# daisy9542/yolo-puncture

Hardware: AMD Instinct MI355X
Metric: images/sec (higher is better)
Workload: dtype bf16

## Files before the change

### include/yolop.h

```cpp
#ifndef YOLOP_H
#define YOLOP_H

#include <stddef.h>
#include <stdint.h>

#ifdef __cplusplus
extern "C" {
#endif

#define YP_OK 0
#define YP_ERR_ARG -1
#define YP_ERR_STATE -2
#define YP_ERR_HIP -3
#define YP_ERR_WEIGHT -4

#define YP_BF16 0
#define YP_F32 1

#define YP_TASK_DETECT 0
#define YP_TASK_SEGMENT 1

#define YP_NM 32
#define YP_MAX_MASKS 480
#define YP_MAX_DET 512
// ... 83 lines not shown

typedef struct yp_cls yp_cls;
int yp_cls_create(int variant, int dtype, int device, yp_cls** out);
int yp_cls_destroy(yp_cls* e);
int yp_cls_weight_count(const yp_cls* e);
int yp_cls_weight_info(const yp_cls* e, int i, char* name, int name_cap, int64_t shape[4], int* ndim);
int yp_cls_set_weight(yp_cls* e, const char* name, const float* host, const int64_t* shape, int ndim);
int yp_cls_finalize(yp_cls* e);
int yp_cls_forward(yp_cls* e, const uint8_t* frames_dev, int B, int H, int W, int bgr, const int32_t* boxes_dev, float* logits_out,
                   float* prob_out, int32_t* cls_out, void* stream);
int yp_cls_set_graph(yp_cls* e, int enable);
int yp_cls_tensor_count(const yp_cls* e);
int yp_cls_tensor_info(const yp_cls* e, int i, char* name, int name_cap, int dims[4] );
int yp_cls_tensor_read(yp_cls* e, int i, float* host_out);

typedef struct yp_comm yp_comm;
int yp_comm_unique_id(void* id128);
int yp_comm_create(const void* id128, int rank, int world, int device, yp_comm** out);
int yp_allgather(yp_comm* c, const void* send_dev, void* recv_dev, size_t bytes_per_rank, void* stream);
int yp_comm_destroy(yp_comm* c);

#define YP_MAX_ANCHORS 294912
int yp_max_batch(const yp_engine* e, int H, int W);
int yp_plan(yp_engine* e, int B, int H, int W);
int yp_op_info(const yp_engine* e, int i, char* name, int name_cap, int* kind, double* flops,
               double* bytes);
int yp_op_kernel(const yp_engine* e, int i, char* name, int name_cap);
int yp_op_output(const yp_engine* e, int i, int* tensor, int* coff, int* C);
int yp_op_input(const yp_engine* e, int i, int* tensor, int* coff, int* C, int* c_read);
int yp_op_fusion(const yp_engine* e, int i, int* pre, int* pre_stored);
int yp_debug_op_form(const yp_engine* e, int i, int* form, int* absorbed, int cap);
int yp_run_op(yp_engine* e, int i, const uint8_t* in_dev, float* det_out, int32_t* idx_out, float* coeff_out, void* stream);
int yp_tensor_write(yp_engine* e, int tensor, int coff, int C, const float* host);
int yp_tensor_count(const yp_engine* e);
int yp_tensor_info(const yp_engine* e, int i, char* name, int name_cap, int dims[4] , int* is_f32);
int yp_tensor_read(yp_engine* e, int i, float* host_out);

int yp_profile(yp_engine* e, const uint8_t* in_dev, int B, int H, int W, float* det_out, int32_t* idx_out,
               float* coeff_out, float* ms_out, int iters, void* stream);

int yp_set_nms(yp_engine* e, float conf, float iou);

int yp_set_attention_form(yp_engine* e, int form);

int yp_set_autotune(yp_engine* e, int enable);

int yp_tuning_export(const yp_engine* e, int32_t* cfg_out, int cap);
int yp_tuning_import(yp_engine* e, int B, int H, int W, const int32_t* cfg, int n);

int yp_debug_force_conv_cfg(int cfg);
int yp_debug_op_cfg(const yp_engine* e, int i, int* cfg);
int yp_debug_last_store_form(void);
int yp_debug_max_workgroups(int n);
int yp_debug_conv_families(int* base, int* num_cfgs, int cap);
int yp_debug_ablation(int v);
int yp_debug_head_clocks(uint64_t* out8);
int yp_debug_attention(const void* qkv_dev, void* o_dev, int dtype, int B, int N, int nh, int kd, int hd, int q_stride, int q_coff, int o_stride,
                       int o_coff, int wgs, int* kernel_out, void* stream);
int yp_debug_attention_form(const void* qkv_dev, void* o_dev, int dtype, int B, int N, int nh, int kd, int hd, int q_stride, int q_coff, int o_stride,
                            int o_coff, int wgs, int form, int* kernel_out, void* stream);
int yp_debug_topk_anchors(const uint32_t* const mk_dev[3], int B, const int hw[3][2], int k, int32_t* sel_out_dev, uint32_t* thr_out_dev, void* stream);
int yp_debug_head_branch_clocks(uint64_t* out8);
int yp_debug_head_winners(yp_engine* e, int32_t* sel_host, float* box_host, float* coeff_host);
int yp_debug_contour_clocks(uint64_t* out12);
int yp_debug_pwsp_clocks(uint64_t* out32);

int yp_tuning_source(const yp_engine* e);

int yp_debug_host_selftest(yp_engine* e);
int yp_debug_graph_info(const yp_engine* e, int64_t* out6);
int yp_debug_head_positions(yp_engine* e, int64_t* out6);
int yp_debug_marker(void* stream);

int yp_set_graph(yp_engine* e, int enable);

#ifdef __cplusplus
}
#endif
#endif
```

### yolo-puncture_amd/csrc/common.h

```cpp
#pragma once
#include <hip/hip_runtime.h>
#include <stdint.h>
#include <atomic>
#include <cstdlib>
#include <string>
#include <vector>

namespace yp {

enum DType { DT_BF16 = 0, DT_F32 = 1 };
enum Act { ACT_NONE = 0, ACT_SILU = 1, ACT_RELU = 2 };

enum OpKind {
    OP_STEM = 0,
    OP_CONV = 1,
    OP_DWCONV = 2,
    OP_POOL5 = 3,
    OP_UPSAMPLE = 4,
    OP_ATTN = 5,
    OP_HEAD = 6,
    OP_CONVT = 7,
    OP_AMAX = 9,
    OP_POOL3 = 8,
};
// ... 103 lines not shown
    const float* bias;
    void* y; int y_stride, y_coff; int Ho, Wo;
    const void* res; int res_stride, res_coff;
    int B, ks, stride, pad, act;
    int gs, gstride;
    size_t x_bytes;
};

struct StemParams {
    const uint8_t* x; int H, W;
    const float* w;
    const void* wpk;
    const float* bias;
    void* y; int y_stride, y_coff; int Ho, Wo, C0; int B;
    int act;
};

struct FrontParams {
    const uint8_t* img; int imgH, imgW, B;
    const void* w0; const float* bias0; int act0, C0; int H1, W1;
    const void* w1; const float* bias1; int act1, C1, Kpad1; size_t w1_bytes;
    const void* w2; const float* bias2; int act2, C2, Kpad2; size_t w2_bytes;
    void* y; int y_stride, y_coff; size_t y_bytes; int Ho, Wo;
    unsigned long long* clk;
};
bool frontend_valid(const FrontParams& p);
hipError_t launch_frontend(const FrontParams& p, hipStream_t st);

struct C2fParams {
    const void* x; int x_stride, x_coff; size_t x_bytes;
    int B, H, W, C;
    const void* w1; const float* bias1; int act1, Kpad1; size_t w1_bytes;
    const void* w2; const float* bias2; int act2, Kpad2; size_t w2_bytes;
    int shortcut;
    const void* w3; const float* bias3; int act3, Kpad3, Cout; size_t w3_bytes;
    void* y; int y_stride, y_coff; size_t y_bytes;
    unsigned long long* clk;
    int wide;
};
bool c2f_fused_valid(const C2fParams& p);

struct ScdParams {
    const void* x; int x_stride, x_coff; size_t x_bytes; int B, H, W, K;
    const void* w1; const float* bias1; int act1, Kpad1, C; size_t w1_bytes;
    const void* wd; const float* biasd; int actd;
    void* y; int y_stride, y_coff; size_t y_bytes; int Ho, Wo;
    unsigned long long* clk;
};
bool scdown_fused_valid(const ScdParams& p);
const char* scdown_fused_kernel_name(const ScdParams& p);
bool scdown_stream_valid(const ScdParams& p);
const char* scdown_stream_kernel_name(const ScdParams& p);
hipError_t launch_scdown_stream(const ScdParams& p, hipStream_t st);
hipError_t launch_scdown_fused(const ScdParams& p, hipStream_t st);
hipError_t launch_c2f_fused(const C2fParams& p, hipStream_t st);

struct PoolParams {
    const void* x; int x_stride, x_coff;
    void* y; int y_stride, y_coff;
    int B, H, W, C;
};

struct UpParams {
    const void* x; int x_stride, x_coff;
    void* y; int y_stride, y_coff;
    int B, H, W, C;
};

struct AttnParams {
    const void* qkv; int q_stride, q_coff;
    void* o; int o_stride, o_coff;
    int B, N, nh, kd, hd;
    float scale;
};

struct HeadParams {
    const float* box[3]; const float* cls[3]; const float* cf[3];
    int hw[3][2]; int nlev;
    int B, nc, max_det, A;
    float* det; int32_t* idx; float* coeff;
    void* scratch;
    const unsigned* mk[3];
    const float* nms_params;
    float* nms_ws;
    int* sp_sel; int* sp_wlist; int* sp_wcount; unsigned* sp_thr; float* sp_box; float* sp_cf;
    int* sp_plist; int* sp_pcount; int sp_plist_off[3], sp_plist_cap[3];
};
hipError_t launch_head_stage1(const HeadParams& p, hipStream_t st);
hipError_t launch_head_stage2(const HeadParams& p, hipStream_t st);
constexpr int HEAD_MAXK = 512;
struct HeadBranchParams {
    const void* x[3]; int x_stride[3], x_coff[3], H[3], W[3], Cin[3]; size_t x_bytes[3];
    const void* w0[3]; int Kpad0[3]; const float* b0[3];
    const void* w1[3]; int Kpad1[3]; const float* b1[3];
    const void* w2[3]; int Kpad2[3]; const float* b2[3];
    int act0, act1;
    int B, max_det, maxk, cmid, cout;
    int A0, A1;
    const int* sel;
    const int* wlist;
    const int* wcount;
    float* out;
    const int* plist; const int* pcount;
    int plist_off[3], plist_cap[3];
    void* t0; size_t t0_off[3], t0_bytes;
    int pos_grid;
// ... 206 lines not shown
```

### yolo-puncture_amd/csrc/engine.hip

```cpp
#include "../../include/yolop.h"
#include "common.h"
#include <algorithm>
#include <array>
#include <chrono>

#include <cmath>
#include <cstdarg>
#include <cstdio>
#include <cstring>
#include <cstdlib>
#include <dlfcn.h>
#include <fcntl.h>
#include <fstream>
#include <map>
#include <sstream>
#include <memory>

using namespace yp;

static thread_local char g_err[512] = "";
static int fail(int code, const char* fmt, ...) {
    va_list ap;
    va_start(ap, fmt);
    vsnprintf(g_err, sizeof(g_err), fmt, ap);
// ... 2390 lines not shown
    HIPCHK(hipSetDevice(e->device));
    HIPCHK(hipDeviceSynchronize());
    const SparseWs ws = sparse_ws_layout(*e);
    const char* base = (const char*)e->sp_ws;
    int pc[8];
    HIPCHK(hipMemcpy(pc, base + ws.pcount, sizeof(pc), hipMemcpyDeviceToHost));
    std::vector<int> wc((size_t)e->pB * 3);
    HIPCHK(hipMemcpy(wc.data(), base + ws.wcount, wc.size() * 4, hipMemcpyDeviceToHost));
    for (int l = 0; l < 3; ++l) {
        out6[l] = std::min(pc[4 + l], ws.plist_cap[l]);
        for (int b = 0; b < e->pB; ++b) out6[3 + l] += wc[(size_t)b * 3 + l];
    }
    return 1;
}

__global__ void op_marker_kernel(int* sink) { if (sink) *sink = 0; }
int yp_debug_marker(void* stream) {
    hipLaunchKernelGGL(op_marker_kernel, dim3(1), dim3(1), 0, (hipStream_t)stream, (int*)nullptr);
    HIPCHK(hipGetLastError());
    return YP_OK;
}

int yp_debug_pwsp_clocks(uint64_t* out32) {
    if (!out32) return fail(YP_ERR_ARG, "yp_debug_pwsp_clocks: null output");
    HIPCHK(hipDeviceSynchronize());
    HIPCHK(pwsp_read_clocks((unsigned long long*)out32));
    return YP_OK;
}

int yp_debug_contour_clocks(uint64_t* out12) {
    if (!out12) return fail(YP_ERR_ARG, "yp_debug_contour_clocks: null output");
    HIPCHK(hipDeviceSynchronize());
    HIPCHK(contour_read_clocks((unsigned long long*)out12));
    return YP_OK;
}

int yp_debug_ablation(int v) {
    conv_set_debug_ablation(v);
    return 0;
}

int yp_debug_force_conv_cfg(int cfg) {
    conv_dma_force_cfg(cfg);
    return conv_dma_family.num_cfgs;
}

int yp_debug_last_store_form(void) {
    store_form_watched().store(true);
    return last_store_form().exchange(-1);
}

int yp_debug_max_workgroups(int n) { return debug_max_workgroups_ref().exchange(n > 0 ? n : 0); }

int yp_debug_op_cfg(const yp_engine* e, int i, int* cfg) {
    if (!e || i < 0 || i >= (int)e->ops.size() || !cfg) return fail(YP_ERR_ARG, "bad argument");
    *cfg = op_launch_cfg(*e, e->ops[i]);
    return YP_OK;
}

int yp_debug_conv_families(int* base, int* num_cfgs, int cap) {
    for (int f = 0; f < kNumConvFamilies && f < cap; ++f) {
        if (base) base[f] = kConvFamilies[f]->base;
        if (num_cfgs) num_cfgs[f] = kConvFamilies[f]->num_cfgs;
    }
    return kNumConvFamilies;
}

int yp_debug_host_selftest(yp_engine* e) {
    if (!e) return fail(YP_ERR_ARG, "null engine");
    if (!e->planned) return fail(YP_ERR_STATE, "yp_plan has not been called");
    size_t acc = 0;
    if (!e->finalized)
        for (WeightDesc& w : e->weights) {
            if (!w.have_w || !w.have_b || w.w.empty()) continue;
            std::vector<unsigned char> main, aux;
            pack_weight(*e, w, main, aux);
            acc += main.size() + aux.size();
        }
    for (const Op& o : e->ops) {
        if (o.skip) continue;
        if (fused(o)) build_form_params(*e, o);
        else if (o.kind == OP_CONV) acc += (size_t)conv_params(*e, o).Cout;
    }
    save_tune_cache(*e);
    (void)load_tune_cache(*e);
    {
        const std::string tp = tune_cache_path(*e, true);
        if (!tp.empty() && std::ifstream(tp).good()) {
            std::vector<std::pair<int, std::string>> keep;
            for (const Op& o : e->ops) keep.emplace_back(o.cfg, o.kernel);
            const bool ok = load_tune_cache(*e, true);
            for (size_t i = 0; i < e->ops.size(); ++i) { e->ops[i].cfg = keep[i].first; e->ops[i].kernel = keep[i].second; }
            if (!ok) return fail(YP_ERR_STATE, "packaged tune table %s does not apply to this build's plan", tp.c_str());
        }
    }
    remember_tuning(*e);
    if (!recall_tuning(*e)) return fail(YP_ERR_STATE, "internal: tuning memo lost");
    int rc = build_lane_schedule(*e);
    if (rc != YP_OK) return rc;
    std::vector<char> rec(e->ops.size(), 0);
    std::vector<char> seen(e->n_lanes, 0);
    seen[0] = 1;
    for (const auto& stp : e->lane_steps) {
        const Op& o = e->ops[stp.op];
        for (int j : stp.waits)
            if (!rec[j]) return fail(YP_ERR_STATE, "internal: %s waits on %s, which never records", o.name.c_str(), e->ops[j].name.c_str());
// ... 264 lines not shown
```

### yolo-puncture_amd/csrc/scdown_fused.hip

```cpp
#include "common.h"
#include <cstdio>
#include <cstdlib>
#include <vector>

namespace yp {

constexpr int SD_NW = 8;
constexpr int SD_TH = 4, SD_TW = 8;
constexpr int SD_RH = 2 * SD_TH + 1, SD_RW = 2 * SD_TW + 1;
constexpr int SD_RP = SD_RH * SD_RW;
constexpr int SD_XP = 39;
constexpr int SD_XB = SD_XP * 1024;
constexpr int SD_TB = 160 * 128;
constexpr int SD_WB = 64 * 256;
constexpr int SD_LDS = 2 * SD_XB + 2 * SD_TB + 2 * SD_WB + 5120 + 2048;

__global__ __launch_bounds__(SD_NW * 64) void scdown_fused_kernel(const ScdParams p, const int tiles_h, const int tiles_w, const int G) {
    extern __shared__ __attribute__((aligned(1024))) unsigned char smem[];
    unsigned char* const Xs = smem;
    unsigned char* const Ts = Xs + 2 * SD_XB;
    unsigned char* const Ws = Ts + 2 * SD_TB;
    unsigned char* const Wd = Ws + 2 * SD_WB;
    float* const Bs = (float*)(Wd + 5120);

// ... 109 lines not shown
            SD_STAMP(3)

            {
                bf16x8 wA[4], xB[2][5];
                int q[5];
#pragma unroll
                for (int kc = 0; kc < 4; ++kc) { const int row = cf * 16 + fr; wA[kc] = *(const bf16x8*)(Wg + row * 256 + (((kc * 4 + fc) ^ (row & 15)) * 16)); }
#pragma unroll
                for (int j = 0; j < 5; ++j) { const int qq = (ps + 2 * j) * 16 + fr; q[j] = qq < SD_XP * 4 ? qq : SD_XP * 4 - 1; }
                auto rd = [&](int kc) {
#pragma unroll
                    for (int j = 0; j < 5; ++j) xB[kc & 1][j] = *(const bf16x8*)(X + q[j] * 256 + (((kc * 4 + fc) ^ (q[j] & 15)) * 16));
                };
                f32x4 acc[5];
                const f32x4 b1 = *(const f32x4*)(Bs + g * 64 + cf * 16 + fc * 4);
#pragma unroll
                for (int j = 0; j < 5; ++j) acc[j] = b1;
                rd(0);
                __builtin_amdgcn_sched_barrier(0);
#pragma unroll
                for (int kc = 0; kc < 4; ++kc) {
                    if (kc < 3) rd(kc + 1);
#pragma unroll
                    for (int j = 0; j < 5; ++j) acc[j] = __builtin_amdgcn_mfma_f32_16x16x32_bf16(wA[kc], xB[kc & 1][j], acc[j], 0, 0, 0);
                    __builtin_amdgcn_sched_barrier(0);
                }
#pragma unroll
                for (int j = 0; j < 5; ++j) {
                    const int qq = (ps + 2 * j) * 16 + fr;
                    const int py = q[j] / SD_RW, px = q[j] - py * SD_RW;
                    const int iy = 2 * th * SD_TH - 1 + py, ix = 2 * tw * SD_TW - 1 + px;
                    const bool in = (unsigned)iy < (unsigned)p.H && (unsigned)ix < (unsigned)p.W;
                    float v[4] = {acc[j][0], acc[j][1], acc[j][2], acc[j][3]};
                    if (p.act1 == ACT_SILU) silu4_packed(v);
                    __attribute__((aligned(8))) __bf16 ob[4];
#pragma unroll
                    for (int i = 0; i < 4; ++i) ob[i] = (__bf16)(in ? v[i] : 0.f);
                    const int ch = cf * 16 + fc * 4;
                    lds_write8(Tg + qq * 128 + (((ch >> 3) ^ ((qq >> 1) & 7)) * 16) + (ch & 7) * 2, *(const unsigned long long*)ob);
                }
            }
            asm volatile("s_waitcnt lgkmcnt(0)" ::: "memory");
            SD_STAMP(2)
            pg = g; pb = b; pth = th; ptw = tw;
        }
    }
    __builtin_amdgcn_s_barrier();
    if (pg >= 0) dw_stage(Ts + ((gi - 1) & 1) * SD_TB, pg, pb, pth, ptw);
    __builtin_amdgcn_s_waitcnt(0 | (7 << 4) | (0xF << 8));
    if (p.clk && lane == 0)
        for (int i = 0; i < 4; ++i) p.clk[((size_t)blockIdx.x * SD_NW + wave) * 4 + i] = clk[i];
}

const char* scdown_fused_kernel_name(const ScdParams& p) { return scdown_stream_valid(p) ? scdown_stream_kernel_name(p) : "scdown_fused_kernel"; }

bool scdown_fused_valid(const ScdParams& p) {
    if (scdown_stream_valid(p)) return true;
    if (p.K != 128 || p.Kpad1 != 128 || (p.C & 63) || p.C > 256 || p.C < 64) return false;
    if ((p.x_stride & 7) || (p.x_coff & 7) || (p.y_stride & 3) || (p.y_coff & 3)) return false;
    if (p.x_bytes >= (1ull << 31) || p.y_bytes >= (1ull << 31)) return false;
    if (p.w1_bytes < (size_t)p.C * p.Kpad1 * 2) return false;
    if ((p.H & 1) || (p.W & 1) || p.Ho * 2 != p.H || p.Wo * 2 != p.W) return false;
    const long covered = (long)((p.Ho + SD_TH - 1) / SD_TH * SD_TH) * ((p.Wo + SD_TW - 1) / SD_TW * SD_TW);
    if (covered * 2 > (long)p.Ho * p.Wo * 3) return false;
    return true;
}

hipError_t launch_scdown_fused(const ScdParams& p, hipStream_t st) {
    if (scdown_stream_valid(p)) return launch_scdown_stream(p, st);
    const int tiles_h = (p.Ho + SD_TH - 1) / SD_TH, tiles_w = (p.Wo + SD_TW - 1) / SD_TW;
    const int num_tiles = p.B * tiles_h * tiles_w;
    int G = 256;
    if (G > num_tiles) G = num_tiles;
    static size_t granted = 0;
    if (hipError_t e = allow_dynamic_lds((const void*)scdown_fused_kernel, (size_t)SD_LDS, granted)) return e;
    static const bool clocks = env_on("YOLOP_SCD_CLOCKS");
    if (clocks) {
        ScdParams q = p;
        const size_t n = (size_t)G * SD_NW * 4;
        if (hipMalloc((void**)&q.clk, n * 8) != hipSuccess) return hipErrorOutOfMemory;
        hipLaunchKernelGGL(scdown_fused_kernel, dim3(G), dim3(SD_NW * 64), (size_t)SD_LDS, st, q, tiles_h, tiles_w, G);
        (void)hipStreamSynchronize(st);
        std::vector<unsigned long long> h(n);
        (void)hipMemcpy(h.data(), q.clk, n * 8, hipMemcpyDeviceToHost);
        (void)hipFree(q.clk);
        static const char* nm[4] = {"wait", "barrier", "G (1x1+SiLU)", "issue+D (dw)"};
        const double steps = (double)num_tiles / G * (p.C / 64);
        for (int w = 0; w < SD_NW; w += SD_NW - 1) {
            fprintf(stderr, "[scdown clocks] wave %d, s_memtime ticks per channel group:", w);
            for (int i = 0; i < 4; ++i) {
                double s = 0;
                for (int g = 0; g < G; ++g) s += (double)h[((size_t)g * SD_NW + w) * 4 + i];
                fprintf(stderr, " %s %.0f", nm[i], s / G / steps);
            }
            fprintf(stderr, "\n");
        }
        return hipGetLastError();
    }
    hipLaunchKernelGGL(scdown_fused_kernel, dim3(G), dim3(SD_NW * 64), (size_t)SD_LDS, st, p, tiles_h, tiles_w, G);
    return hipGetLastError();
}

}
```

### yolo-puncture_amd/engine.py

```python
from __future__ import annotations

import ctypes as C
import os
from typing import Dict, List, Optional, Tuple

import numpy as np
import torch

from .weights import fold_state

_LIB: Optional[C.CDLL] = None
_HERE = os.path.dirname(os.path.abspath(__file__))
LIB_PATH = os.environ.get("YOLOP_LIB") or os.path.join(_HERE, "libyolop.so")

YP_BF16, YP_F32 = 0, 1
TASK_DETECT, TASK_SEGMENT = 0, 1
OP_KINDS = {0: "stem", 1: "conv", 2: "dwconv", 3: "pool5", 4: "upsample", 5: "attn", 6: "head", 7: "convT", 8: "pool3", 9: "amax"}
FORMS = ("plain", "dwpw", "dwpw_tail", "s2pw", "frontend", "c2f", "scdown", "pwsp", "cls_out")


class ModelDesc(C.Structure):
    _fields_ = [("variant", C.c_int), ("nc", C.c_int), ("task", C.c_int), ("dtype", C.c_int), ("max_det", C.c_int), ("family", C.c_int)]


# ... 27 lines not shown
    lib.yp_mask_contours.restype = C.c_int
    lib.yp_mask_contours_scaled.argtypes = [vp, C.c_int, C.c_int, C.c_int, C.c_int, C.c_int, vp, vp, vp, C.c_int, vp, C.c_int, C.c_int, vp]
    lib.yp_mask_contours_scaled.restype = C.c_int
    lib.yp_mask_contours_large_workspace.argtypes = [C.c_int, C.c_int, C.c_int]
    lib.yp_mask_contours_large_workspace.restype = C.c_size_t
    lib.yp_mask_contours_large.argtypes = [vp, C.c_int, C.c_int, C.c_int, C.c_int, C.c_int, vp, vp, vp, C.c_int, vp, C.c_int, C.c_int, C.c_int, vp,
                                           C.c_size_t, vp]
    lib.yp_mask_contours_large.restype = C.c_int
    lib.yp_plan.argtypes = [vp, C.c_int, C.c_int, C.c_int]
    lib.yp_max_batch.argtypes = [vp, C.c_int, C.c_int]
    lib.yp_max_batch.restype = C.c_int
    lib.yp_debug_topk_anchors.argtypes = [C.POINTER(vp), C.c_int, C.POINTER(C.c_int), C.c_int, vp, vp, vp]
    lib.yp_debug_topk_anchors.restype = C.c_int
    lib.yp_debug_attention.argtypes = [vp, vp] + [C.c_int] * 11 + [ip, vp]
    lib.yp_debug_attention.restype = C.c_int
    lib.yp_debug_attention_form.argtypes = [vp, vp] + [C.c_int] * 12 + [ip, vp]
    lib.yp_debug_attention_form.restype = C.c_int
    lib.yp_set_attention_form.argtypes = [vp, C.c_int]
    lib.yp_set_attention_form.restype = C.c_int
    lib.yp_op_info.argtypes = [vp, C.c_int, C.c_char_p, C.c_int, ip, C.POINTER(C.c_double), C.POINTER(C.c_double)]
    lib.yp_op_output.argtypes = [vp, C.c_int, ip, ip, ip]
    lib.yp_op_kernel.argtypes = [vp, C.c_int, C.c_char_p, C.c_int]
    lib.yp_op_fusion.argtypes = [vp, C.c_int, ip, ip]
    lib.yp_op_fusion.restype = C.c_int
    lib.yp_debug_op_form.argtypes = [vp, C.c_int, ip, ip, C.c_int]
    lib.yp_debug_op_form.restype = C.c_int
    lib.yp_run_op.argtypes = [vp, C.c_int, vp, vp, vp, vp, vp]
    lib.yp_tensor_write.argtypes = [vp, C.c_int, C.c_int, C.c_int, vp]
    lib.yp_tensor_count.argtypes = [vp]
    lib.yp_tensor_info.argtypes = [vp, C.c_int, C.c_char_p, C.c_int, ip, ip]
    lib.yp_tensor_read.argtypes = [vp, C.c_int, vp]
    lib.yp_profile.argtypes = [vp, vp, C.c_int, C.c_int, C.c_int, vp, vp, vp, vp, C.c_int, vp]
    lib.yp_set_graph.argtypes = [vp, C.c_int]
    lib.yp_set_autotune.argtypes = [vp, C.c_int]
    lib.yp_set_nms.argtypes = [vp, C.c_float, C.c_float]
    lib.yp_set_nms.restype = C.c_int
    lib.yp_debug_host_selftest.argtypes = [vp]
    lib.yp_debug_host_selftest.restype = C.c_int
    lib.yp_tuning_source.argtypes = [vp]
    lib.yp_tuning_source.restype = C.c_int
    lib.yp_debug_graph_info.argtypes = [vp, C.POINTER(C.c_int64)]
    lib.yp_debug_graph_info.restype = C.c_int
    lib.yp_debug_head_positions.argtypes = [vp, C.POINTER(C.c_int64)]
    lib.yp_debug_head_positions.restype = C.c_int
    lib.yp_debug_marker.argtypes = [vp]
    lib.yp_debug_marker.restype = C.c_int
    lib.yp_debug_force_conv_cfg.argtypes = [C.c_int]
    lib.yp_debug_op_cfg.argtypes = [vp, C.c_int, ip]
    lib.yp_debug_op_cfg.restype = C.c_int
    lib.yp_debug_last_store_form.argtypes = []
    lib.yp_debug_last_store_form.restype = C.c_int
    lib.yp_debug_max_workgroups.argtypes = [C.c_int]
    lib.yp_debug_max_workgroups.restype = C.c_int
    lib.yp_debug_conv_families.argtypes = [ip, ip, C.c_int]
    lib.yp_debug_conv_families.restype = C.c_int
    lib.yp_debug_ablation.argtypes = [C.c_int]
    lib.yp_debug_head_clocks.argtypes = [C.POINTER(C.c_uint64)]
    lib.yp_debug_head_branch_clocks.argtypes = [C.POINTER(C.c_uint64)]
    lib.yp_debug_contour_clocks.argtypes = [C.POINTER(C.c_uint64)]
    lib.yp_debug_pwsp_clocks.argtypes = [C.POINTER(C.c_uint64)]
    lib.yp_letterbox.argtypes = [vp, C.c_int, C.c_int, vp] + [C.c_int] * 7 + [vp]
    lib.yp_letterbox.restype = C.c_int
    lib.yp_letterbox_batch.argtypes = [vp, C.c_int, C.c_int, C.c_int, vp] + [C.c_int] * 7 + [vp]
    lib.yp_letterbox_batch.restype = C.c_int
    lib.yp_masks_frames.argtypes = [vp, vp, C.c_int, vp, C.c_long, vp, C.c_int, C.c_int, vp, vp]
    lib.yp_masks_frames.restype = C.c_int
    lib.yp_masks_frames_input.argtypes = [vp, vp, C.c_int, vp, C.c_long, vp, C.c_int, C.c_int, vp, vp]
    lib.yp_masks_frames_input.restype = C.c_int
    lib.yp_comm_unique_id.argtypes = [vp]
    lib.yp_comm_create.argtypes = [vp, C.c_int, C.c_int, C.c_int, C.POINTER(vp)]
    lib.yp_allgather.argtypes = [vp, vp, vp, C.c_size_t, vp]
    lib.yp_comm_destroy.argtypes = [vp]
    for fn in ("yp_comm_unique_id", "yp_comm_create", "yp_allgather", "yp_comm_destroy"):
        getattr(lib, fn).restype = C.c_int
    for fn in ("yp_create", "yp_destroy", "yp_weight_count", "yp_weight_info", "yp_set_weight", "yp_finalize",
               "yp_forward", "yp_proto", "yp_masks", "yp_plan", "yp_op_info", "yp_op_output", "yp_op_input", "yp_tensor_count",
               "yp_tensor_info", "yp_tensor_read", "yp_profile", "yp_set_graph", "yp_run_op", "yp_tensor_write",
               "yp_op_kernel", "yp_set_autotune", "yp_debug_force_conv_cfg", "yp_debug_ablation"):
        getattr(lib, fn).restype = C.c_int
    if path is None:
        _LIB = lib
    return lib


EXPORTS = ["yp_last_error", "yp_create", "yp_destroy", "yp_weight_count", "yp_weight_info", "yp_set_weight",
           "yp_finalize", "yp_forward", "yp_proto", "yp_masks", "yp_id_mask_resized", "yp_plan", "yp_op_info", "yp_op_output", "yp_op_input", "yp_op_fusion",
           "yp_tensor_count", "yp_tensor_info", "yp_tensor_read", "yp_profile", "yp_set_graph", "yp_run_op",
           "yp_tensor_write", "yp_op_kernel", "yp_set_autotune", "yp_tuning_export", "yp_tuning_import", "yp_set_nms", "yp_debug_force_conv_cfg", "yp_debug_op_cfg", "yp_debug_op_form", "yp_debug_last_store_form", "yp_debug_max_workgroups", "yp_debug_conv_families", "yp_debug_ablation", "yp_debug_head_clocks", "yp_debug_head_branch_clocks", "yp_debug_head_winners", "yp_debug_contour_clocks", "yp_debug_pwsp_clocks", "yp_debug_host_selftest", "yp_debug_graph_info", "yp_tuning_source", "yp_debug_head_positions", "yp_debug_marker", "yp_max_batch", "yp_debug_topk_anchors", "yp_debug_attention", "yp_debug_attention_form", "yp_set_attention_form", "yp_letterbox", "yp_letterbox_batch", "yp_masks_frames", "yp_masks_frames_input", "yp_mask_contours",
           "yp_mask_contours_scaled", "yp_mask_contours_large_workspace", "yp_mask_contours_large", "yp_comm_unique_id", "yp_comm_create", "yp_allgather", "yp_comm_destroy",
           "yp_u2net_create", "yp_u2net_destroy", "yp_u2net_weight_count", "yp_u2net_weight_info", "yp_u2net_set_weight", "yp_u2net_finalize",
           "yp_u2net_forward", "yp_u2net_forward_crops", "yp_u2net_set_graph", "yp_u2net_tensor_count", "yp_u2net_tensor_info", "yp_u2net_tensor_read",
           "yp_u2net_op_count", "yp_u2net_op_info",
           "yp_cls_create", "yp_cls_destroy", "yp_cls_weight_count", "yp_cls_weight_info", "yp_cls_set_weight", "yp_cls_finalize",
           "yp_cls_forward", "yp_cls_set_graph", "yp_cls_tensor_count", "yp_cls_tensor_info", "yp_cls_tensor_read"]


MAX_ANCHORS = 294912
ATTENTION_FORMS = {"auto": 0, "stream": 1, "stream_wide": 3}


def _attention_form(form) -> int:
    if form not in ATTENTION_FORMS:
        raise ValueError(f"attention form {form!r}: one of {sorted(ATTENTION_FORMS)}")
    return ATTENTION_FORMS[form]


def topk_anchors(mk: List[torch.Tensor], hw, k: int) -> Tuple[torch.Tensor, torch.Tensor]:
    lib = load_library()
    if len(mk) != 3 or len(hw) != 3:
        raise ValueError("three levels")
    B = int(mk[0].shape[0])
    dev = mk[0].device
    for t, (h, w) in zip(mk, hw):
        if t.dtype != torch.int32 or not t.is_contiguous() or t.device != dev or tuple(t.shape) != (B, int(h) * int(w)):
            raise ValueError("mk[l] must be contiguous int32 [B, H_l * W_l] on one device")
    sel = torch.full((B, 512), -1, dtype=torch.int32, device=dev)
    thr = torch.zeros((B,), dtype=torch.int32, device=dev)
    ptrs = (C.c_void_p * 3)(*[t.data_ptr() for t in mk])
    hwa = (C.c_int * 6)(*[int(v) for pair in hw for v in pair])
    rc = lib.yp_debug_topk_anchors(ptrs, B, hwa, int(k), C.c_void_p(sel.data_ptr()), C.c_void_p(thr.data_ptr()), C.c_void_p(_stream_ptr(dev)))
    if rc < 0:
        raise YolopError(lib.yp_last_error().decode())
    return sel, thr


def attention(qkv: torch.Tensor, nh: int, kd: int, hd: int, q_coff: int = 0, out: Optional[torch.Tensor] = None, o_coff: int = 0,
              wgs: int = 0, form: str = "auto") -> Tuple[torch.Tensor, int]:
    lib = load_library()
    if qkv.dim() != 3 or qkv.dtype not in (torch.bfloat16, torch.float32) or not qkv.is_contiguous() or not qkv.is_cuda:
        raise ValueError("qkv must be a contiguous device bf16 / float32 [B, N, q_stride]")
    B, N, q_stride = (int(v) for v in qkv.shape)
    if out is None:
        out = torch.empty((B, N, int(nh) * int(hd)), dtype=qkv.dtype, device=qkv.device)
    if out.dim() != 3 or out.dtype != qkv.dtype or not out.is_contiguous() or out.device != qkv.device or tuple(out.shape[:2]) != (B, N):
        raise ValueError("out must be a contiguous [B, N, o_stride] of qkv's dtype on its device")
    kernel = C.c_int(-1)
    rc = lib.yp_debug_attention_form(C.c_void_p(qkv.data_ptr()), C.c_void_p(out.data_ptr()), YP_BF16 if qkv.dtype == torch.bfloat16 else YP_F32, B, N,
                                int(nh), int(kd), int(hd), q_stride, int(q_coff), int(out.shape[2]), int(o_coff), int(wgs), _attention_form(form), C.byref(kernel),
                                C.c_void_p(_stream_ptr(qkv.device)))
    if rc < 0:
        raise YolopError(lib.yp_last_error().decode())
# ... 427 lines not shown
```

Baseline: 23370.

## Add band-streaming fused SCDown kernel for 1x1 conv plus stride-2 depthwise

Adds a new fused SCDown kernel. Each workgroup owns a horizontal band of output rows and a 64-channel slice. It streams pairs of input rows into LDS with async buffer loads, computes the 1x1 conv with MFMA into a 4-row ring buffer in LDS, then applies the 3x3 stride-2 depthwise conv from that ring, so the intermediate tensor never goes to global memory. The kernel is chosen ahead of the existing stream and chunked variants for specific shapes (K=128,W=80 and K=256,W=40) when enough workgroups result. The cost is recomputing one halo row per band plus extra debug entry points.

```diff
diff --git a/include/yolop.h b/include/yolop.h
--- a/include/yolop.h
+++ b/include/yolop.h
@@ -159,6 +159,10 @@
 int yp_debug_op_cfg(const yp_engine* e, int i, int* cfg);
 int yp_debug_last_store_form(void);
 int yp_debug_max_workgroups(int n);
+int yp_debug_scd_bands(int n);
+int yp_debug_scdown(const void* x_dev, const void* w1_dev, const float* b1_dev, const void* wd_dev, const float* bd_dev, void* t_dev, void* y_dev,
+                    int B, int H, int W, int K, int C, int x_stride, int x_coff, int y_stride, int y_coff, int act1, int actd, int form, int bands,
+                    void* stream);
 int yp_debug_conv_families(int* base, int* num_cfgs, int cap);
 int yp_debug_ablation(int v);
 int yp_debug_head_clocks(uint64_t* out8);
diff --git a/yolo-puncture_amd/csrc/common.h b/yolo-puncture_amd/csrc/common.h
--- a/yolo-puncture_amd/csrc/common.h
+++ b/yolo-puncture_amd/csrc/common.h
@@ -179,6 +179,13 @@
 bool scdown_stream_valid(const ScdParams& p);
 const char* scdown_stream_kernel_name(const ScdParams& p);
 hipError_t launch_scdown_stream(const ScdParams& p, hipStream_t st);
+bool scdown_band_supported(const ScdParams& p);
+bool scdown_band_valid(const ScdParams& p);
+int scdown_band_bands(const ScdParams& p);
+size_t scdown_band_lds_bytes(const ScdParams& p);
+const char* scdown_band_kernel_name(const ScdParams& p);
+hipError_t launch_scdown_band(const ScdParams& p, hipStream_t st);
+int scdown_band_debug_bands(int n);
 hipError_t launch_scdown_fused(const ScdParams& p, hipStream_t st);
 hipError_t launch_c2f_fused(const C2fParams& p, hipStream_t st);
 
diff --git a/yolo-puncture_amd/csrc/engine.hip b/yolo-puncture_amd/csrc/engine.hip
--- a/yolo-puncture_amd/csrc/engine.hip
+++ b/yolo-puncture_amd/csrc/engine.hip
@@ -2466,6 +2466,52 @@
 
 int yp_debug_max_workgroups(int n) { return debug_max_workgroups_ref().exchange(n > 0 ? n : 0); }
 
+int yp_debug_scd_bands(int n) { return scdown_band_debug_bands(n); }
+
+int yp_debug_scdown(const void* x_dev, const void* w1_dev, const float* b1_dev, const void* wd_dev, const float* bd_dev, void* t_dev, void* y_dev,
+                    int B, int H, int W, int K, int C, int x_stride, int x_coff, int y_stride, int y_coff, int act1, int actd, int form, int bands,
+                    void* stream) {
+    if (!x_dev || !w1_dev || !b1_dev || !wd_dev || !bd_dev || !y_dev || (form == 0 && !t_dev)) return fail(YP_ERR_ARG, "yp_debug_scdown: null argument");
+    if (form < 0 || form > 2) return fail(YP_ERR_ARG, "yp_debug_scdown: form = %d (0 separate kernels | 1 band | 2 band, host side only)", form);
+    if (B < 1 || H < 2 || W < 2 || (H & 1) || (W & 1) || K < 32 || (K & 31) || C < 128 || (C & 127) || x_coff < 0 || y_coff < 0 || x_coff + K > x_stride ||
+        y_coff + C > y_stride || (act1 != ACT_NONE && act1 != ACT_SILU) || (actd != ACT_NONE && actd != ACT_SILU) || bands < 0)
+        return fail(YP_ERR_ARG, "yp_debug_scdown: bad size (B %d, H %d, W %d, K %d, C %d, x %d+%d, y %d+%d, act %d %d, bands %d)", B, H, W, K, C, x_stride, x_coff,
+                    y_stride, y_coff, act1, actd, bands);
+    if ((int64_t)B * H * W * std::max(std::max(x_stride, y_stride), C) * 2 >= (1ll << 31)) return fail(YP_ERR_ARG, "yp_debug_scdown: a buffer of 2^31 bytes or more");
+    ScdParams p{};
+    p.x = x_dev; p.x_stride = x_stride; p.x_coff = x_coff; p.x_bytes = (size_t)B * H * W * x_stride * 2; p.B = B; p.H = H; p.W = W; p.K = K;
+    p.w1 = w1_dev; p.bias1 = b1_dev; p.act1 = act1; p.Kpad1 = K; p.C = C; p.w1_bytes = (size_t)C * K * 2;
+    p.wd = wd_dev; p.biasd = bd_dev; p.actd = actd;
+    p.y = y_dev; p.y_stride = y_stride; p.y_coff = y_coff; p.Ho = H / 2; p.Wo = W / 2; p.y_bytes = (size_t)B * p.Ho * p.Wo * y_stride * 2;
+    hipStream_t st = (hipStream_t)stream;
+    hipError_t err;
+    if (form >= 1 && !scdown_band_supported(p)) return fail(YP_ERR_ARG, "yp_debug_scdown: the band kernel does not support this shape");
+    if (form == 2) return (int)scdown_band_lds_bytes(p);
+    if (form == 1) {
+        const int was = scdown_band_debug_bands(bands);
+        err = launch_scdown_band(p, st);
+        scdown_band_debug_bands(was);
+    } else {
+        ConvParams c{};
+        c.x = x_dev; c.x_stride = x_stride; c.x_coff = x_coff; c.H = H; c.W = W; c.Cin = K;
+        c.w = w1_dev; c.Kpad = K; c.bias = b1_dev;
+        c.y = t_dev; c.y_stride = C; c.y_coff = 0; c.Ho = H; c.Wo = W; c.Cout = C;
+        c.M = B * H * W; c.ks = 1; c.stride = 1; c.pad = 0; c.act = act1;
+        c.up = 1; c.x_bytes = p.x_bytes; c.w_bytes = p.w1_bytes; c.y_bytes = (size_t)B * H * W * C * 2; c.cfg = -1;
+        DwParams d{};
+        d.x = t_dev; d.x_stride = C; d.x_coff = 0; d.H = H; d.W = W; d.C = C;
+        d.w = wd_dev; d.bias = bd_dev;
+        d.y = y_dev; d.y_stride = y_stride; d.y_coff = y_coff; d.Ho = p.Ho; d.Wo = p.Wo;
+        d.B = B; d.ks = 3; d.stride = 2; d.pad = 1; d.act = actd;
+        d.x_bytes = c.y_bytes;
+        err = launch_conv(c, DT_BF16, st);
+        if (err == hipSuccess) err = launch_dwconv(d, DT_BF16, st);
+    }
+    if (err == hipSuccess) err = hipStreamSynchronize(st);
+    if (err != hipSuccess) return fail(YP_ERR_HIP, "yp_debug_scdown: %s", hipGetErrorString(err));
+    return YP_OK;
+}
+
 int yp_debug_op_cfg(const yp_engine* e, int i, int* cfg) {
     if (!e || i < 0 || i >= (int)e->ops.size() || !cfg) return fail(YP_ERR_ARG, "bad argument");
     *cfg = op_launch_cfg(*e, e->ops[i]);
diff --git a/yolo-puncture_amd/csrc/scdown_band.hip b/yolo-puncture_amd/csrc/scdown_band.hip
--- /dev/null
+++ b/yolo-puncture_amd/csrc/scdown_band.hip
@@ -0,0 +1,217 @@
+#include "common.h"
+#include <cstdlib>
+
+namespace yp {
+
+constexpr int SB_NW = 8;
+constexpr int SB_NS = 64;
+constexpr int SB_PB = SB_NS * 2;
+
+__device__ __forceinline__ unsigned ring_off(int q, int ch) {
+    const int p = q ^ ((q >> 1) & 1);
+    return (unsigned)(p * SB_PB + ((((ch >> 3) ^ p) & 7) << 4) + ((((ch >> 2) ^ (p >> 3)) & 1) << 3));
+}
+
+template <int NKS, int FPW>
+__global__ __launch_bounds__(SB_NW * 64) void scdown_band_kernel(const ScdParams p, const int bands, const int slices, const int RW) {
+    constexpr int RB = NKS * 64;
+    constexpr int PXC = 2 * FPW * 16;
+    constexpr int XB = PXC * RB;
+    constexpr int PPW = XB / 1024 / SB_NW;
+    constexpr int CPR = RB / 16;
+    constexpr int NST = (FPW * 8 + 31) / 32;
+    extern __shared__ __attribute__((aligned(1024))) unsigned char smem[];
+    unsigned char* const Xs = smem;
+    unsigned char* const Ts = smem + 2 * XB;
+    const int tid = threadIdx.x, lane = tid & 63;
+    const int wave = __builtin_amdgcn_readfirstlane(tid >> 6);
+    const int fr = lane & 15, fc = lane >> 4;
+    const int cf = wave & 3, ph = wave >> 2;
+
+    int bid = xcd_remap(blockIdx.x, gridDim.x);
+    const int c0 = (bid % slices) * SB_NS; bid /= slices;
+    const int band = bid % bands;
+    const int b = bid / bands;
+    const int r0 = band * p.Ho / bands, r1 = (band + 1) * p.Ho / bands;
+    const int s0 = r0 > 0 ? r0 - 1 : 0;
+    const int P = 2 * p.W;
+
+    const __amdgpu_buffer_rsrc_t xrs = __builtin_amdgcn_make_buffer_rsrc((void*)p.x, 0, (int)p.x_bytes, 0x00020000);
+    const __amdgpu_buffer_rsrc_t wrs = __builtin_amdgcn_make_buffer_rsrc((void*)p.w1, 0, (int)p.w1_bytes, 0x00020000);
+    const __amdgpu_buffer_rsrc_t yrs = __builtin_amdgcn_make_buffer_rsrc((void*)p.y, 0, (int)p.y_bytes, 0x00020000);
+
+    auto issue_step = [&](int s, int slot) {
+        unsigned char* const dst = Xs + slot * XB;
+        const int pix0 = (b * p.H + 2 * s) * p.W;
+#pragma unroll
+        for (int j = 0; j < PPW; ++j) {
+            const int ii = wave + j * SB_NW;
+            const int q = ii * 64 + lane;
+            const int px = q / CPR, pc = q - px * CPR;
+            const int c = pc ^ (px & 15);
+            const bool ok = s < r1 && px < P;
+            const unsigned voff = ok ? (unsigned)(((pix0 + px) * p.x_stride + p.x_coff + c * 8) * 2) : kBufferOOB;
+            __builtin_amdgcn_raw_ptr_buffer_load_lds(xrs, (lds_void*)(dst + ii * 1024), 16, voff, 0, 0, 0);
+        }
+    };
+    issue_step(s0, 0);
+
+    bf16x8 wreg[NKS];
+    float b1[4];
+    {
+        const int row = c0 + cf * 16 + fr;
+#pragma unroll
+        for (int ks = 0; ks < NKS; ++ks) {
+            const unsigned voff = (unsigned)((row * p.Kpad1 + (ks >> 1) * 64 + fc * 16 + (ks & 1) * 8) * 2);
+            const __attribute__((ext_vector_type(4))) unsigned v = __builtin_amdgcn_raw_buffer_load_b128(wrs, voff, 0, 0);
+            wreg[ks] = __builtin_bit_cast(bf16x8, v);
+        }
+#pragma unroll
+        for (int r = 0; r < 4; ++r) b1[r] = p.bias1[c0 + cf * 16 + fc * 4 + r];
+    }
+    const int dc = (tid & 15) * 4, xg = tid >> 4;
+    f32x2 wd[9][2], bd[2];
+    {
+#pragma unroll
+        for (int t = 0; t < 9; ++t) {
+            const uint2 u = *(const uint2*)((const __bf16*)p.wd + t * p.C + c0 + dc);
+            wd[t][0] = f32x2{__uint_as_float(u.x << 16), __uint_as_float(u.x & 0xffff0000u)};
+            wd[t][1] = f32x2{__uint_as_float(u.y << 16), __uint_as_float(u.y & 0xffff0000u)};
+        }
+        bd[0] = f32x2{p.biasd[c0 + dc], p.biasd[c0 + dc + 1]};
+        bd[1] = f32x2{p.biasd[c0 + dc + 2], p.biasd[c0 + dc + 3]};
+    }
+    for (int i = tid; i < 4 * RW * SB_PB / 8; i += SB_NW * 64) lds_write8(Ts + i * 8, 0ull);
+    wait_vmcnt<0>();
+#pragma unroll
+    for (int ks = 0; ks < NKS; ++ks) asm volatile("" : "+v"(wreg[ks]));
+#pragma unroll
+    for (int r = 0; r < 4; ++r) asm volatile("" : "+v"(b1[r]));
+#pragma unroll
+    for (int t = 0; t < 9; ++t) { asm volatile("" : "+v"(wd[t][0])); asm volatile("" : "+v"(wd[t][1])); }
+    asm volatile("" : "+v"(bd[0]));
+    asm volatile("" : "+v"(bd[1]));
+    asm volatile("s_waitcnt lgkmcnt(0)" ::: "memory");
+
+    const unsigned ts_l = lds_addr(Ts);
+    const int slot_b = RW * SB_PB;
+    for (int s = s0, it = 0; s < r1; ++s, ++it) {
+        if (it == 0) wait_vmcnt<0>();
+        else wait_vmcnt<NST>();
+        __builtin_amdgcn_s_barrier();
+        const int slot = it & 1;
+        issue_step(s + 1, slot ^ 1);
+        {
+            f32x4 acc[FPW];
+#pragma unroll
+            for (int j = 0; j < FPW; ++j) acc[j] = f32x4{b1[0], b1[1], b1[2], b1[3]};
+            const unsigned char* const X = Xs + slot * XB;
+#pragma unroll
+            for (int ks = 0; ks < NKS; ++ks) {
+                const int ch = (ks >> 1) * 8 + fc * 2 + (ks & 1);
+                bf16x8 xf[FPW];
+#pragma unroll
+                for (int j = 0; j < FPW; ++j) xf[j] = *(const bf16x8*)(X + ((ph + 2 * j) * 16 + fr) * RB + ((ch ^ fr) << 4));
+#pragma unroll
+                for (int j = 0; j < FPW; ++j) acc[j] = __builtin_amdgcn_mfma_f32_16x16x32_bf16(wreg[ks], xf[j], acc[j], 0, 0, 0);
+            }
+#pragma unroll
+            for (int j = 0; j < FPW; ++j) {
+                const int px = (ph + 2 * j) * 16 + fr;
+                const int r = px >= p.W ? 1 : 0;
+                const int col = px - r * p.W;
+                float v[4] = {acc[j][0], acc[j][1], acc[j][2], acc[j][3]};
+                if (p.act1 == ACT_SILU) silu4_packed(v);
+                const u32x2 o = pack_bf16x4(v);
+                const unsigned dst = ts_l + (unsigned)(((2 * s + r) & 3) * slot_b) + ring_off(col + 1, cf * 16 + fc * 4);
+                if (px < P) asm volatile("ds_write_b64 %0, %1" : : "v"(dst), "v"(__builtin_bit_cast(unsigned long long, o)) : "memory");
+            }
+        }
+        asm volatile("s_waitcnt lgkmcnt(0)" ::: "memory");
+        __builtin_amdgcn_s_barrier();
+#pragma unroll
+        for (int n = 0; n < NST; ++n) {
+            const int ox = xg + 32 * n;
+            const int oxc = ox < p.Wo ? ox : p.Wo - 1;
+            unsigned long long tv[9];
+#pragma unroll
+            for (int ky = 0; ky < 3; ++ky) {
+                const unsigned char* const T = Ts + ((2 * s - 1 + ky) & 3) * slot_b;
+#pragma unroll
+                for (int kx = 0; kx < 3; ++kx) tv[ky * 3 + kx] = lds_read8_async(T + ring_off(2 * oxc + kx, dc));
+            }
+            asm volatile("s_waitcnt lgkmcnt(0)" : "+v"(tv[0]), "+v"(tv[1]), "+v"(tv[2]), "+v"(tv[3]), "+v"(tv[4]), "+v"(tv[5]), "+v"(tv[6]), "+v"(tv[7]), "+v"(tv[8])::"memory");
+            f32x2 a0 = bd[0], a1 = bd[1];
+#pragma unroll
+            for (int t = 0; t < 9; ++t) {
+                const unsigned lo = (unsigned)tv[t], hi = (unsigned)(tv[t] >> 32);
+                a0 = __builtin_elementwise_fma(f32x2{__uint_as_float(lo << 16), __uint_as_float(lo & 0xffff0000u)}, wd[t][0], a0);
+                a1 = __builtin_elementwise_fma(f32x2{__uint_as_float(hi << 16), __uint_as_float(hi & 0xffff0000u)}, wd[t][1], a1);
+            }
+            float v[4] = {a0[0], a0[1], a1[0], a1[1]};
+            if (p.actd == ACT_SILU) silu4_packed(v);
+            const bool ok = s >= r0 && ox < p.Wo;
+            const unsigned off = ok ? (unsigned)((((b * p.Ho + s) * p.Wo + ox) * p.y_stride + p.y_coff + c0 + dc) * 2) : kBufferOOB;
+            store_bf16x4(v, yrs, off);
+        }
+    }
+    wait_vmcnt<0>();
+}
+
+size_t scdown_band_lds_bytes(const ScdParams& p) {
+    const int fpw = p.K == 128 ? 5 : 3;
+    return (size_t)2 * (2 * fpw * 16) * p.K * 2 + (size_t)4 * ((p.W + 4) & ~3) * SB_PB;
+}
+
+static std::atomic<int>& band_debug_ref() { static std::atomic<int> v{0}; return v; }
+int scdown_band_debug_bands(int n) { return band_debug_ref().exchange(n > 0 ? n : 0); }
+
+int scdown_band_bands(const ScdParams& p) {
+    const int dbg = band_debug_ref().load(std::memory_order_relaxed);
+    if (dbg) return dbg < p.Ho ? dbg : p.Ho;
+    const int slices = p.C / SB_NS;
+    int bands = 256 / (p.B * slices);
+    if (bands > p.Ho / 4) bands = p.Ho / 4;
+    return bands < 1 ? 1 : bands;
+}
+
+bool scdown_band_supported(const ScdParams& p) {
+    if (p.clk) return false;
+    if ((p.K != 128 && p.K != 256) || p.Kpad1 != p.K || p.C < SB_NS || (p.C % SB_NS) || p.C > 512) return false;
+    if ((p.x_stride & 7) || (p.x_coff & 7) || (p.y_stride & 3) || (p.y_coff & 3)) return false;
+    if (p.x_bytes >= (1ull << 31) || p.y_bytes >= (1ull << 31) || p.w1_bytes >= (1ull << 31)) return false;
+    if (p.w1_bytes < (size_t)p.C * p.Kpad1 * 2) return false;
+    if (p.act1 != ACT_SILU && p.act1 != ACT_NONE) return false;
+    if (p.actd != ACT_SILU && p.actd != ACT_NONE) return false;
+    if (p.B < 1 || p.H < 2 || p.W < 2 || (p.H & 1) || (p.W & 1) || p.Ho * 2 != p.H || p.Wo * 2 != p.W) return false;
+    if (2 * p.W > 2 * (p.K == 128 ? 5 : 3) * 16) return false;
+    return scdown_band_lds_bytes(p) <= 160 * 1024;
+}
+
+bool scdown_band_valid(const ScdParams& p) {
+    static const bool off = env_on("YOLOP_NO_SCD_BAND");
+    if (off || !scdown_band_supported(p)) return false;
+    if (band_debug_ref().load(std::memory_order_relaxed)) return true;
+    if (!((p.K == 128 && p.W == 80) || (p.K == 256 && p.W == 40))) return false;
+    return p.B * scdown_band_bands(p) * (p.C / SB_NS) >= 128;
+}
+
+const char* scdown_band_kernel_name(const ScdParams& p) { return p.K == 128 ? "scdown_fused_kernel<band,4>" : "scdown_fused_kernel<band,8>"; }
+
+template <int NKS, int FPW>
+static hipError_t launch_scdown_band_t(const ScdParams& p, hipStream_t st) {
+    const size_t sh = scdown_band_lds_bytes(p);
+    auto kern = scdown_band_kernel<NKS, FPW>;
+    static size_t granted = 0;
+    if (hipError_t e = allow_dynamic_lds((const void*)kern, sh, granted)) return e;
+    const int bands = scdown_band_bands(p), slices = p.C / SB_NS;
+    hipLaunchKernelGGL(kern, dim3((unsigned)(p.B * bands * slices)), dim3(SB_NW * 64), sh, st, p, bands, slices, (p.W + 4) & ~3);
+    return hipGetLastError();
+}
+
+hipError_t launch_scdown_band(const ScdParams& p, hipStream_t st) {
+    if (!scdown_band_supported(p)) return hipErrorInvalidValue;
+    return p.K == 128 ? launch_scdown_band_t<4, 5>(p, st) : launch_scdown_band_t<8, 3>(p, st);
+}
+
+}
diff --git a/yolo-puncture_amd/csrc/scdown_fused.hip b/yolo-puncture_amd/csrc/scdown_fused.hip
--- a/yolo-puncture_amd/csrc/scdown_fused.hip
+++ b/yolo-puncture_amd/csrc/scdown_fused.hip
@@ -185,10 +185,11 @@
         for (int i = 0; i < 4; ++i) p.clk[((size_t)blockIdx.x * SD_NW + wave) * 4 + i] = clk[i];
 }
 
-const char* scdown_fused_kernel_name(const ScdParams& p) { return scdown_stream_valid(p) ? scdown_stream_kernel_name(p) : "scdown_fused_kernel"; }
-
-bool scdown_fused_valid(const ScdParams& p) {
-    if (scdown_stream_valid(p)) return true;
+const char* scdown_fused_kernel_name(const ScdParams& p) {
+    return scdown_band_valid(p) ? scdown_band_kernel_name(p) : scdown_stream_valid(p) ? scdown_stream_kernel_name(p) : "scdown_fused_kernel";
+}
+
+static bool scdown_chunked_valid(const ScdParams& p) {
     if (p.K != 128 || p.Kpad1 != 128 || (p.C & 63) || p.C > 256 || p.C < 64) return false;
     if ((p.x_stride & 7) || (p.x_coff & 7) || (p.y_stride & 3) || (p.y_coff & 3)) return false;
     if (p.x_bytes >= (1ull << 31) || p.y_bytes >= (1ull << 31)) return false;
@@ -199,8 +200,12 @@
     return true;
 }
 
+bool scdown_fused_valid(const ScdParams& p) { return scdown_band_valid(p) || scdown_stream_valid(p) || scdown_chunked_valid(p); }
+
 hipError_t launch_scdown_fused(const ScdParams& p, hipStream_t st) {
+    if (scdown_band_valid(p)) return launch_scdown_band(p, st);
     if (scdown_stream_valid(p)) return launch_scdown_stream(p, st);
+    if (!scdown_chunked_valid(p)) return hipErrorInvalidValue;
     const int tiles_h = (p.Ho + SD_TH - 1) / SD_TH, tiles_w = (p.Wo + SD_TW - 1) / SD_TW;
     const int num_tiles = p.B * tiles_h * tiles_w;
     int G = 256;
diff --git a/yolo-puncture_amd/engine.py b/yolo-puncture_amd/engine.py
--- a/yolo-puncture_amd/engine.py
+++ b/yolo-puncture_amd/engine.py
@@ -103,6 +103,10 @@
     lib.yp_debug_last_store_form.restype = C.c_int
     lib.yp_debug_max_workgroups.argtypes = [C.c_int]
     lib.yp_debug_max_workgroups.restype = C.c_int
+    lib.yp_debug_scd_bands.argtypes = [C.c_int]
+    lib.yp_debug_scd_bands.restype = C.c_int
+    lib.yp_debug_scdown.argtypes = [C.c_void_p] * 7 + [C.c_int] * 13 + [C.c_void_p]
+    lib.yp_debug_scdown.restype = C.c_int
     lib.yp_debug_conv_families.argtypes = [ip, ip, C.c_int]
     lib.yp_debug_conv_families.restype = C.c_int
     lib.yp_debug_ablation.argtypes = [C.c_int]
@@ -137,7 +141,7 @@
 EXPORTS = ["yp_last_error", "yp_create", "yp_destroy", "yp_weight_count", "yp_weight_info", "yp_set_weight",
            "yp_finalize", "yp_forward", "yp_proto", "yp_masks", "yp_id_mask_resized", "yp_plan", "yp_op_info", "yp_op_output", "yp_op_input", "yp_op_fusion",
            "yp_tensor_count", "yp_tensor_info", "yp_tensor_read", "yp_profile", "yp_set_graph", "yp_run_op",
-           "yp_tensor_write", "yp_op_kernel", "yp_set_autotune", "yp_tuning_export", "yp_tuning_import", "yp_set_nms", "yp_debug_force_conv_cfg", "yp_debug_op_cfg", "yp_debug_op_form", "yp_debug_last_store_form", "yp_debug_max_workgroups", "yp_debug_conv_families", "yp_debug_ablation", "yp_debug_head_clocks", "yp_debug_head_branch_clocks", "yp_debug_head_winners", "yp_debug_contour_clocks", "yp_debug_pwsp_clocks", "yp_debug_host_selftest", "yp_debug_graph_info", "yp_tuning_source", "yp_debug_head_positions", "yp_debug_marker", "yp_max_batch", "yp_debug_topk_anchors", "yp_debug_attention", "yp_debug_attention_form", "yp_set_attention_form", "yp_letterbox", "yp_letterbox_batch", "yp_masks_frames", "yp_masks_frames_input", "yp_mask_contours",
+           "yp_tensor_write", "yp_op_kernel", "yp_set_autotune", "yp_tuning_export", "yp_tuning_import", "yp_set_nms", "yp_debug_force_conv_cfg", "yp_debug_op_cfg", "yp_debug_op_form", "yp_debug_last_store_form", "yp_debug_max_workgroups", "yp_debug_scd_bands", "yp_debug_scdown", "yp_debug_conv_families", "yp_debug_ablation", "yp_debug_head_clocks", "yp_debug_head_branch_clocks", "yp_debug_head_winners", "yp_debug_contour_clocks", "yp_debug_pwsp_clocks", "yp_debug_host_selftest", "yp_debug_graph_info", "yp_tuning_source", "yp_debug_head_positions", "yp_debug_marker", "yp_max_batch", "yp_debug_topk_anchors", "yp_debug_attention", "yp_debug_attention_form", "yp_set_attention_form", "yp_letterbox", "yp_letterbox_batch", "yp_masks_frames", "yp_masks_frames_input", "yp_mask_contours",
            "yp_mask_contours_scaled", "yp_mask_contours_large_workspace", "yp_mask_contours_large", "yp_comm_unique_id", "yp_comm_create", "yp_allgather", "yp_comm_destroy",
            "yp_u2net_create", "yp_u2net_destroy", "yp_u2net_weight_count", "yp_u2net_weight_info", "yp_u2net_set_weight", "yp_u2net_finalize",
            "yp_u2net_forward", "yp_u2net_forward_crops", "yp_u2net_set_graph", "yp_u2net_tensor_count", "yp_u2net_tensor_info", "yp_u2net_tensor_read",
```

Result: no change. 23580 (median of 6 runs) (+0.9%).
